# leggedrobotics/wild_visual_navigation

Measured on NVIDIA H100. Metric: frames/sec end-to-end (DINO feat + seg + MLP train-step) at 448x448, higher is better.
Workload: dtype bf16 operands / fp32 accumulate (ViT, STEGO head, per-pixel MLP); fp32 (k-means, train step)

## Files before the change

include/wvn_b200.h:

```cpp
#ifndef WVN_B200_H_
#define WVN_B200_H_

#include <stddef.h>
#include <stdint.h>

#ifdef __cplusplus
extern "C" {
#endif

typedef enum {
  WVN_STATUS_OK = 0,
  WVN_STATUS_INVALID = -1,
  WVN_STATUS_CUDA = -2,
  WVN_STATUS_NO_DEVICE = -3,
  WVN_STATUS_STATE = -4
} wvn_status;

const char* wvn_last_error(void);
int wvn_check_device(void);
int wvn_version(void);
long long wvn_launch_count(void);
void wvn_profile_enable(int category_mask);
int wvn_profile_collect(float* host_ms, long long* host_launches);

int wvn_gemm_bf16(const void* a_bf16, long long lda, const void* w_bf16, const float* bias, void* out, long long ldo,
                  int m, int n, int k, int out_kind, int act, int block_n, void* stream);

typedef struct {
  int m, n, k;
  int epi, act;
  int block_n;
  const void* a;
  long long lda;
  const void* w;
  const float* bias;
  void* out;
  long long ldo;
  const float* pos;
  int tokens_in, npad;
  int dim, heads;
  void* q_out;
  void* k_out;
  void* vt_out;
  int feat, trav_col;
  const void* x;
  long long ldx;
  float* trav;
  float* conf;
  float* loss_reco;
  const float* cg_mean;
  const float* cg_std;
  float cg_std_factor;
  int reverse_m;
  int registers;
  const void* residual;
  long long ldr;
} wvn_gemm_ex_args;
int wvn_gemm_bf16_ex(const wvn_gemm_ex_args* args, void* stream);

int wvn_attention_bf16(const void* q, const void* k, const void* vt, void* out, int batch, int heads, int npad,
                       int n_valid, float scale, void* stream);

int wvn_layernorm(const float* x, const float* gamma, const float* beta, void* out_bf16, long long rows, int dim,
                  float eps, void* stream);

typedef struct wvn_vit wvn_vit_t;

typedef struct {
  int image_size;
  int patch_size;
  int dim;
  int depth;
  int heads;
  int mlp_dim;
  int max_batch;
  int chunk;
  float ln_eps;
  int head_out;
  int registers;
} wvn_vit_config;

int wvn_vit_create(const wvn_vit_config* cfg, wvn_vit_t** out);
void wvn_vit_destroy(wvn_vit_t* h);

int wvn_vit_set_weight(wvn_vit_t* h, const char* name, const float* data, long long numel);

int wvn_vit_forward(wvn_vit_t* h, const float* img, int batch, int in_h, int in_w, int resized_h, int resized_w,
                    float* tokens_out, void* stream);

int wvn_vit_forward_tta(wvn_vit_t* h, const float* img, int batch, int in_h, int in_w, int resized_h, int resized_w,
                        float* tokens_out, void* stream);

int wvn_vit_forward_u8(wvn_vit_t* h, const unsigned char* img_hwc, int batch, int in_h, int in_w, int resized_h,
                       int resized_w, float* tokens_out, void* stream);

int wvn_vit_stego_head(wvn_vit_t* h, int batch, float* out, void* stream);
int wvn_vit_npad(const wvn_vit_t* h);

typedef struct wvn_resnet wvn_resnet_t;

typedef struct {
  int image_size;
  int depth;
  int max_batch;
} wvn_resnet_config;

int wvn_resnet_create(const wvn_resnet_config* cfg, wvn_resnet_t** out);
void wvn_resnet_destroy(wvn_resnet_t* h);
size_t wvn_resnet_workspace_bytes(const wvn_resnet_t* h);
int wvn_resnet_set_weight(wvn_resnet_t* h, const char* name, const float* data, long long numel);
int wvn_resnet_forward(wvn_resnet_t* h, const float* img, int batch, void* const* taps, void* stream);
// ... 160 lines not shown
```

wild_visual_navigation_b200/_C.py:

```python
from __future__ import annotations

import ctypes
import os
from ctypes import POINTER, Structure, byref, c_char_p, c_float, c_int, c_longlong, c_size_t, c_void_p

import torch

_HERE = os.path.dirname(os.path.abspath(__file__))
LIB_PATH = os.environ.get("WVN_B200_LIB", os.path.join(_HERE, "libwvn_b200.so"))


class WvnError(RuntimeError):
    pass


class VitConfig(Structure):
    _fields_ = [
        ("image_size", c_int), ("patch_size", c_int), ("dim", c_int), ("depth", c_int), ("heads", c_int),
        ("mlp_dim", c_int), ("max_batch", c_int), ("chunk", c_int), ("ln_eps", c_float), ("head_out", c_int),
        ("registers", c_int),
    ]


class GemmExArgs(Structure):
    _fields_ = [
        ("m", c_int), ("n", c_int), ("k", c_int), ("epi", c_int), ("act", c_int), ("block_n", c_int),
        ("a", c_void_p), ("lda", c_longlong), ("w", c_void_p), ("bias", c_void_p), ("out", c_void_p), ("ldo", c_longlong),
        ("pos", c_void_p), ("tokens_in", c_int), ("npad", c_int), ("dim", c_int), ("heads", c_int),
        ("q_out", c_void_p), ("k_out", c_void_p), ("vt_out", c_void_p),
        ("feat", c_int), ("trav_col", c_int), ("x", c_void_p), ("ldx", c_longlong), ("trav", c_void_p),
        ("conf", c_void_p), ("loss_reco", c_void_p), ("cg_mean", c_void_p), ("cg_std", c_void_p),
        ("cg_std_factor", c_float), ("reverse_m", c_int), ("registers", c_int), ("residual", c_void_p), ("ldr", c_longlong),
    ]


class ResnetConfig(Structure):
    _fields_ = [("image_size", c_int), ("depth", c_int), ("max_batch", c_int)]


class TrainConfig(Structure):
    _fields_ = [
        ("w_trav", c_float), ("w_reco", c_float), ("std_factor", c_float), ("anomaly_balanced", c_int),
        ("lr", c_float), ("beta1", c_float), ("beta2", c_float), ("eps", c_float),
    ]


class FlowBuffers(Structure):
    _fields_ = [("mask0", c_void_p), ("mask1", c_void_p), ("p1", c_void_p), ("invp1", c_void_p), ("p3", c_void_p),
                ("invp3", c_void_p)]


_lib = None

_P, _I, _L, _F, _S = c_void_p, c_int, c_longlong, c_float, c_size_t
SIGNATURES = {
    "wvn_last_error": (c_char_p, []),
    "wvn_check_device": (_I, []),
    "wvn_version": (_I, []),
    "wvn_launch_count": (_L, []),
    "wvn_profile_enable": (None, [_I]),
    "wvn_profile_collect": (_I, [_P, _P]),
    "wvn_gemm_bf16": (_I, [_P, _L, _P, _P, _P, _L, _I, _I, _I, _I, _I, _I, _P]),
    "wvn_gemm_bf16_ex": (_I, [POINTER(GemmExArgs), _P]),
    "wvn_attention_bf16": (_I, [_P, _P, _P, _P, _I, _I, _I, _I, _F, _P]),
    "wvn_layernorm": (_I, [_P, _P, _P, _P, _L, _I, _F, _P]),
    "wvn_vit_create": (_I, [POINTER(VitConfig), POINTER(_P)]),
    "wvn_vit_destroy": (None, [_P]),
    "wvn_vit_set_weight": (_I, [_P, c_char_p, _P, _L]),
    "wvn_vit_forward": (_I, [_P, _P, _I, _I, _I, _I, _I, _P, _P]),
    "wvn_vit_forward_u8": (_I, [_P, _P, _I, _I, _I, _I, _I, _P, _P]),
    "wvn_vit_forward_tta": (_I, [_P, _P, _I, _I, _I, _I, _I, _P, _P]),
    "wvn_vit_stego_head": (_I, [_P, _I, _P, _P]),
    "wvn_vit_npad": (_I, [_P]),
    "wvn_resnet_create": (_I, [POINTER(ResnetConfig), POINTER(_P)]),
    "wvn_resnet_destroy": (None, [_P]),
    "wvn_resnet_workspace_bytes": (_S, [_P]),
    "wvn_resnet_set_weight": (_I, [_P, c_char_p, _P, _L]),
    "wvn_resnet_forward": (_I, [_P, _P, _I, _P, _P]),
    "wvn_im2col_bf16_nhwc": (_I, [_P, _I, _I, _I, _I, _I, _I, _I, _P, _L, _P]),
    "wvn_im2col_image": (_I, [_P, _I, _I, _I, _I, _I, _I, _P, _L, _P]),
    "wvn_maxpool3s2_bf16_nhwc": (_I, [_P, _I, _I, _I, _I, _P, _P]),
    "wvn_segment_pool_pyramid": (_I, [_P, _I, _I, _I, _I, _P, _P, _P, _P, _P, _P, _P]),
    "wvn_upsample_dense": (_I, [_P, _P, _I, _I, _I, _I, _I, _I, _P]),
    "wvn_logits_argmax": (_I, [_P, _L, _I, _I, _I, _I, _I, _I, _I, _I, _I, _I, _P, _P, _P]),
    "wvn_flip_average": (_I, [_P, _I, _I, _I, _L, _P]),
    "wvn_stego_kmeans_workspace_bytes": (_S, [_I, _I, _I]),
    "wvn_stego_kmeans": (_I, [_P, _L, _I, _I, _I, _I, _I, _I, _I, _I, _P, _P, _P]),
    "wvn_segment_workspace_bytes": (_S, [_I, _I, _I, _I]),
    "wvn_segment_reduce": (_I, [_P, _I, _I, _I, _I, _P, _I, _I, _I, _P, _P, _P, _P, _I, _P, _P]),
    "wvn_segment_relabel": (_I, [_P, _I, _L, _I, _P, _P, _P]),
    "wvn_supervision_pool": (_I, [_P, _P, _I, _I, _I, _I, _I, _P, _P, _P, _P]),
    "wvn_slic_tables": (None, [_P, _P, _P]),
    "wvn_slic_geometry": (_I, [_I, _I, _I, _P, _P, _P]),
    "wvn_slic_workspace_bytes": (_S, [_I, _I, _I, _I]),
    "wvn_slic": (_I, [_P, _I, _I, _I, _I, _F, _I, _P, _P, _P, _P, _P, _P]),
    "wvn_project_and_render": (_I, [_P, _P, _P, _P, _I, _I, _I, _I, _I, _P, _P, _P, _P, _P, _P]),
    "wvn_mission_propagate_workspace_bytes": (_S, [_I, _I]),
    "wvn_mission_propagate": (_I, [_P, _P, _I, _P, _P, _P, _I, _P, _P, _P, _I, _I, _I, _P, _P, _P, _P, _P]),
    "wvn_mlp_infer_create": (_I, [_I, _I, _I, _I, POINTER(_P)]),
    "wvn_mlp_infer_destroy": (None, [_P]),
    "wvn_mlp_infer_reserve": (_I, [_P, _I]),
    "wvn_mlp_infer_set_params": (_I, [_P, _P, _P]),
    "wvn_mlp_infer_pixels": (_I, [_P, _P, _I, _I, _I, _I, _I, _P, _P, _F, _P, _P, _P]),
    "wvn_mlp_infer_pixels_vit": (_I, [_P, _P, _I, _I, _I, _P, _P, _F, _P, _P, _P]),
    "wvn_mlp_infer_rows": (_I, [_P, _P, _L, _P, _P, _F, _P, _P, _P]),
    "wvn_mlp_infer_create_double": (_I, [_I, _I, _I, _I, POINTER(_P)]),
    "wvn_mlp_param_count": (_S, [_I, _I, _I]),
    "wvn_mlp_train_workspace_bytes": (_S, [_I, _I, _I, _I]),
    "wvn_mlp_train_scalars_bytes": (_S, []),
    "wvn_mlp_train_forward_stats": (_I, [_I, _I, _I, _P, _P, _P, _P, _I, _I, _P, _P, _P]),
    "wvn_mlp_train_backward": (_I, [_I, _I, _I, _P, _P, _P, _P, _I, _I, _L, POINTER(TrainConfig), _P, _P, _P, _P, _P, _P, _P]),
    "wvn_mlp_train_apply": (_I, [_I, _I, _I, _P, _P, _P, _P, _P, _L, POINTER(TrainConfig), _P, _P]),
    "wvn_mlp_train_read_metrics": (_I, [_P, _P, _P]),
    "wvn_mlp_forward_f32": (_I, [_I, _I, _I, _P, _P, _I, _P, _P, _P, _P]),
    "wvn_trainer_destroy": (None, [_P]),
    "wvn_trainer_set_confidence": (_I, [_P, _I, _P, _P, _P, _P, _F, _F]),
# ... 69 lines not shown
```

wild_visual_navigation_b200/csrc/api.cu:

```cuda
#include <cuda_bf16.h>

#include <stdio.h>
#include <stdlib.h>

#include <map>
#include <string>
#include <vector>

#include "../../include/wvn_b200.h"
#include "attention.h"
#include "dense_kernels.h"
#include "double_mlp_train.h"
#include "gcn_train.h"
#include "gemm.h"
#include "host_common.h"
#include "mlp_train.h"
#include "mission_graph.h"
#include "mlp_train_fused.h"
#include "pixel_head.h"
#include "resnet_kernels.h"
#include "segment_kernels.h"
#include "flow_train.h"
#include "footprint_kernels.h"
#include "slic_kernels.h"
// ... 70 lines not shown
  bool forwarded = false;
  int last_batch = 0;

  int add_weight(const std::string& name, long long numel, bool bf16, int cols = 0, int ld = 0) {
    DevBuf b;
    const long long stored = cols > 0 ? numel / cols * ld : numel;
    WVN_PROPAGATE(b.alloc(static_cast<size_t>(stored) * (bf16 ? 2 : 4)));
    owned.push_back(b);
    Weight wt;
    wt.p = b.p; wt.numel = numel; wt.bf16 = bf16; wt.cols = cols; wt.ld = ld;
    w[name] = wt;
    return WVN_OK;
  }
  template <class T>
  T* wp(const std::string& name) { return reinterpret_cast<T*>(w[name].p); }
};

extern "C" {

const char* wvn_last_error(void) { return last_error(); }
int wvn_version(void) { return 108; }

int wvn_check_device(void) {
  int n = 0;
  if (cudaGetDeviceCount(&n) != cudaSuccess || n == 0) return set_error(WVN_ERR_NO_DEVICE, "no CUDA device visible");
  int dev = 0;
  cudaGetDevice(&dev);
  int major = 0;
  cudaDeviceGetAttribute(&major, cudaDevAttrComputeCapabilityMajor, dev);
  int minor = 0;
  cudaDeviceGetAttribute(&minor, cudaDevAttrComputeCapabilityMinor, dev);
  if (major != 9 || minor != 0)
    return set_error(WVN_ERR_NO_DEVICE, "device %d has compute capability %d.%d, need 9.0 (sm_90a)", dev, major, minor);
  return WVN_OK;
}

long long wvn_launch_count(void) { return launch_count(); }
void wvn_profile_enable(int category_mask) { prof_enable(category_mask); }
int wvn_profile_collect(float* host_ms, long long* host_launches) {
  WVN_REQUIRE(host_ms && host_launches, "wvn_profile_collect: null argument");
  return prof_collect(host_ms, host_launches);
}

int wvn_gemm_bf16(const void* a, long long lda, const void* w, const float* bias, void* out, long long ldo, int m, int n,
                  int k, int out_kind, int act, int block_n, void* stream) {
  GemmArgs g;
  g.M = m; g.N = n; g.K = k;
  g.epi = out_kind == 0 ? EPI_BF16 : (out_kind == 1 ? EPI_F32 : EPI_RESID_F32);
  WVN_REQUIRE(out_kind >= 0 && out_kind <= 2, "wvn_gemm_bf16: out_kind %d", out_kind);
  g.act = act; g.bias = bias; g.out = out; g.ldo = ldo;
  return gemm_bf16(g, a, lda, w, block_n, S(stream));
}

int wvn_gemm_bf16_ex(const wvn_gemm_ex_args* x, void* stream) {
  WVN_REQUIRE(x, "wvn_gemm_bf16_ex: null argument");
  GemmArgs g;
  g.M = x->m; g.N = x->n; g.K = x->k; g.epi = x->epi; g.act = x->act;
  g.bias = x->bias; g.out = x->out; g.ldo = x->ldo;
  g.pos = x->pos; g.tokens_in = x->tokens_in; g.npad = x->npad;
  g.dim = x->dim; g.heads = x->heads; g.q = x->q_out; g.k = x->k_out; g.vt = x->vt_out;
  g.feat = x->feat; g.trav_col = x->trav_col; g.x = x->x; g.ldx = x->ldx; g.trav = x->trav; g.conf = x->conf;
  g.loss_reco = x->loss_reco; g.cg_mean = x->cg_mean; g.cg_std = x->cg_std; g.cg_std_factor = x->cg_std_factor;
  g.reverse_m = x->reverse_m; g.registers = x->registers;
  g.residual = x->residual; g.ldr = x->ldr;
  return gemm_bf16(g, x->a, x->lda, x->w, x->block_n, S(stream));
}

int wvn_attention_bf16(const void* q, const void* k, const void* vt, void* out, int batch, int heads, int npad,
                       int n_valid, float scale, void* stream) {
  AttnArgs a;
  a.batch = batch; a.heads = heads; a.npad = npad; a.n_valid = n_valid;
  a.scale_log2 = scale * 1.4426950408889634f;
  a.out = out; a.ldo = static_cast<long long>(heads) * 64;
  return attention_bf16(a, q, k, vt, S(stream));
}

int wvn_layernorm(const float* x, const float* gamma, const float* beta, void* out_bf16, long long rows, int dim,
                  float eps, void* stream) {
  LayerNormArgs a;
  a.rows = rows; a.dim = dim; a.eps = eps;
  return layernorm_rows(x, gamma, beta, out_bf16, nullptr, a, S(stream));
}

int wvn_vit_create(const wvn_vit_config* cfg, wvn_vit_t** out) {
  WVN_REQUIRE(cfg && out, "wvn_vit_create: null argument");
  WVN_PROPAGATE(wvn_check_device());
  WVN_REQUIRE(cfg->dim == 384 || cfg->dim == 768, "vit: dim %d unsupported (384, 768)", cfg->dim);
  WVN_REQUIRE(cfg->heads * 64 == cfg->dim, "vit: heads*64 must equal dim");
  WVN_REQUIRE(cfg->patch_size == 8 || cfg->patch_size == 14 || cfg->patch_size == 16, "vit: patch size %d unsupported",
              cfg->patch_size);
  WVN_REQUIRE(cfg->image_size >= cfg->patch_size, "vit: image size too small");
  WVN_REQUIRE(cfg->mlp_dim % 64 == 0 && cfg->depth > 0 && cfg->max_batch > 0, "vit: bad mlp_dim/depth/max_batch");
  WVN_REQUIRE(cfg->head_out % 64 == 0, "vit: head_out must be a multiple of 64");
  WVN_REQUIRE(cfg->registers >= 0, "vit: registers must be >= 0");
  WVN_REQUIRE(cfg->registers == 0 || cfg->head_out == 0, "vit: register tokens and a STEGO head cannot be combined");
  wvn_vit* h = new wvn_vit();
  h->cfg = *cfg;
  if (h->cfg.ln_eps <= 0.f) h->cfg.ln_eps = 1e-6f;
  h->grid = cfg->image_size / cfg->patch_size;
  h->P = h->grid * h->grid;
  h->t0 = 1 + cfg->registers;
  h->n_valid = h->t0 + h->P;
  h->npad = round_up(h->n_valid, 128);
  h->kpe = 3 * cfg->patch_size * cfg->patch_size;
  h->kpe_ld = patch_pitch(cfg->patch_size);
  h->chunk = cfg->chunk > 0 ? cfg->chunk : 8;
  if (h->chunk > cfg->max_batch) h->chunk = cfg->max_batch;
  const int D = cfg->dim;
  int rc = WVN_OK;
  auto add = [&](const std::string& n, long long numel, bool bf) { if (rc == WVN_OK) rc = h->add_weight(n, numel, bf); };
  add("cls_token", D, false);
  add("pos_embed", static_cast<long long>(1 + h->P) * D, false);
  if (cfg->registers > 0) add("register_tokens", static_cast<long long>(cfg->registers) * D, false);
  if (rc == WVN_OK) rc = h->add_weight("patch_embed.proj.weight", static_cast<long long>(D) * h->kpe, true, h->kpe, h->kpe_ld);
  add("patch_embed.proj.bias", D, false);
  for (int i = 0; i < cfg->depth; ++i) {
    const std::string b = "blocks." + std::to_string(i) + ".";
    add(b + "norm1.weight", D, false);
// ... 1276 lines not shown
```

wild_visual_navigation_b200/csrc/gemm.h:

```cpp
#pragma once

#include <cuda_runtime.h>

namespace wvn {

enum GemmEpilogue : int {
  EPI_BF16 = 0,
  EPI_F32 = 1,
  EPI_RESID_F32 = 2,
  EPI_PATCH = 3,
  EPI_QKV = 4,
  EPI_MLP_HEAD = 5,
  EPI_BF16_RESID = 6,
};

enum GemmAct : int { ACT_NONE = 0, ACT_RELU = 1, ACT_GELU = 2 };

struct GemmArgs {
  int M = 0, N = 0, K = 0;
  int epi = EPI_BF16, act = ACT_NONE;
  const float* bias = nullptr;
  void* out = nullptr;
  long long ldo = 0;
  const float* pos = nullptr;
  int tokens_in = 0;
  int registers = 0;
  int npad = 0;
  int dim = 0, heads = 0;
  void* q = nullptr;
  void* k = nullptr;
  void* vt = nullptr;
  int feat = 0;
  int trav_col = 0;
  const void* x = nullptr;
  long long ldx = 0;
  float* trav = nullptr;
  float* conf = nullptr;
  float* loss_reco = nullptr;
  const float* cg_mean = nullptr;
  const float* cg_std = nullptr;
  float cg_std_factor = 0.5f;
  const void* residual = nullptr;
  long long ldr = 0;
  int max_ctas = 0;
  int reverse_m = 0;
};

int pick_block_n(int N);

inline long long gemm_w_pitch(int K) { return (static_cast<long long>(K) + 7) / 8 * 8; }

int gemm_bf16(const GemmArgs& args, const void* A, long long lda, const void* W, int block_n, cudaStream_t stream);

}
```

wild_visual_navigation_b200/csrc/gemm_wgmma.cu:

```cuda
#include <stdlib.h>

#include <algorithm>

#include "common.cuh"
#include "gemm.h"
#include "host_common.h"

namespace wvn {

namespace {

constexpr int BM = 64;
constexpr int BK = 64;
constexpr int kConsumerWarps = 8;
constexpr int kNumThreads = 128 + kConsumerWarps * 32;
constexpr int kMaxSmemBytes = 227 * 1024;
constexpr int kMaxStages = 8;
constexpr int kFixedSmemBytes = 1024  + 1024 ;
constexpr int kSliceCols = 32;
constexpr int kResidMaxBlockN = 192;

template <bool ROW_OWNER>
struct TileIter {
  int num_m, num_n, m_blk, n_blk, lin;
  __device__ TileIter(int nm, int nn) : num_m(nm), num_n(nn), m_blk(0), n_blk(0), lin(0) {
    if (ROW_OWNER) { m_blk = blockIdx.x; n_blk = 0; }
    else { lin = blockIdx.x; m_blk = lin / num_n; n_blk = lin % num_n; }
  }
  __device__ bool valid() const { return m_blk < num_m; }
  __device__ void next() {
    if (ROW_OWNER) { if (++n_blk == num_n) { n_blk = 0; m_blk += gridDim.x; } }
    else { lin += gridDim.x; m_blk = lin / num_n; n_blk = lin % num_n; }
  }
};

template <int EPI>
constexpr bool kStaged = EPI == EPI_BF16 || EPI == EPI_F32 || EPI == EPI_RESID_F32 || EPI == EPI_QKV || EPI == EPI_BF16_RESID;

template <int BN, int EPI>
struct GemmCfg {
  static constexpr uint32_t kABytes = BM * BK * 2;
  static constexpr uint32_t kBBytes = BN * BK * 2;
  static constexpr uint32_t kStageBytes = kABytes + kBBytes;
  static constexpr uint32_t kSliceBytes = BM * kSliceCols * ((EPI == EPI_F32 || EPI == EPI_RESID_F32) ? 4 : 2);
  static constexpr uint32_t kStagingBytes = kStaged<EPI> ? 2 * 2 * kSliceBytes : 0;
  static constexpr int kStagesRaw = (kMaxSmemBytes - kFixedSmemBytes - kStagingBytes) / kStageBytes;
  static constexpr int kStages = kStagesRaw > kMaxStages ? kMaxStages : kStagesRaw;
  static constexpr uint32_t kSmemBytes = kStages * kStageBytes + kStagingBytes + kFixedSmemBytes;
  static constexpr int kN128 = BN / 128;
  static constexpr int kN64 = (BN % 128) / 64;
  static constexpr int kN32 = (BN % 64) / 32;
};

__device__ __forceinline__ float gelu_erf_fast(float x) {
  const float t = fminf(fabsf(x), 5.5f);
  float p = fmaf(-0.0003865310864f, t, 0.006509808358f);
  p = fmaf(p, t, -0.05048002675f);
  p = fmaf(p, t, -0.4613505006f);
  p = fmaf(p, t, -1.150225043f);
  p = fmaf(p, t, -1.00010848f);
  float e;
  asm("ex2.approx.ftz.f32 %0, %1;" : "=f"(e) : "f"(p));
  return fmaf(-t, e, fmaxf(x, 0.f));
}

template <int ACT>
__device__ __forceinline__ float activate(float v) {
  if (ACT == ACT_RELU) return fmaxf(v, 0.f);
  if (ACT == ACT_GELU) return gelu_erf_fast(v);
  return v;
}

template <int EPI, int ACT, int NREG>
__device__ __forceinline__ void epilogue_frag(const GemmArgs& args, const float (&d)[NREG], const int row0,
                                              const int col_base, const int lane, float (&head_partial)[2]) {
  const int q = lane & 3;
  bool ok[2];
  long long orow[2];
  int tok[2];
#pragma unroll
  for (int h = 0; h < 2; ++h) {
    const int row = row0 + 8 * h;
    ok[h] = row < args.M;
    orow[h] = row;
    tok[h] = 0;
    if (EPI == EPI_PATCH) {
      const int frame = row / args.tokens_in;
      tok[h] = row - frame * args.tokens_in;
      orow[h] = static_cast<long long>(frame) * args.npad + (1 + args.registers) + tok[h];
    }
  }
#pragma unroll
  for (int j = 0; j < NREG / 4; ++j) {
    const int col = col_base + 8 * j + 2 * q;
    float2 b = make_float2(0.f, 0.f);
    if (args.bias != nullptr) b = __ldg(reinterpret_cast<const float2*>(args.bias + col));
#pragma unroll
    for (int h = 0; h < 2; ++h) {
      const float v0 = activate<ACT>(d[4 * j + 2 * h] + b.x), v1 = activate<ACT>(d[4 * j + 2 * h + 1] + b.y);
      if (!ok[h]) continue;
      if (EPI == EPI_PATCH) {
// ... 34 lines not shown
    if (leader) {
      if (si == 0) tma_store_wait_read<0>();
      else tma_store_wait_read<1>();
    }
    named_bar_sync(bar_id, 128);
#pragma unroll
    for (int js = 0; js < 4; ++js) {
      const int j = 4 * s + js;
      const int c = col + 8 * js + 2 * q;
      float2 b = make_float2(0.f, 0.f);
      if (args.bias != nullptr) b = __ldg(reinterpret_cast<const float2*>(args.bias + c));
#pragma unroll
      for (int h = 0; h < 2; ++h) {
        const int r = row_local + 8 * h;
        float a0 = d[4 * j + 2 * h] + b.x, a1 = d[4 * j + 2 * h + 1] + b.y;
        if (EPI == EPI_BF16_RESID && row_tile + r < args.M) {
          const uint32_t rv = __ldg(reinterpret_cast<const uint32_t*>(
              reinterpret_cast<const __nv_bfloat16*>(args.residual) + static_cast<long long>(row_tile + r) * args.ldr + c));
          a0 += bf16_lo(rv);
          a1 += bf16_hi(rv);
        }
        const float v0 = activate<ACT>(a0), v1 = activate<ACT>(a1);
        if (EPI == EPI_F32 || EPI == EPI_RESID_F32) {
          sts64(buf + r * 128 + ((((2 * js + (q >> 1)) ^ (r & 7))) << 4) + (q & 1) * 8, v0, v1);
        } else if (EPI == EPI_QKV && which == 2) {
          const int dd = 8 * js + 2 * q;
          const uint32_t t = 2 * r;
          sts16(buf + dd * 128 + (((t >> 4) ^ (dd & 7)) << 4) + (t & 15), __float2bfloat16_rn(v0));
          sts16(buf + (dd + 1) * 128 + (((t >> 4) ^ ((dd + 1) & 7)) << 4) + (t & 15), __float2bfloat16_rn(v1));
        } else {
          sts32(buf + r * 64 + ((js ^ ((r >> 1) & 3)) << 4) + q * 4, pack_bf16x2(v0, v1));
        }
      }
    }
    fence_proxy_async_smem();
    named_bar_sync(bar_id, 128);
    if (leader) {
      if (EPI == EPI_BF16 || EPI == EPI_F32 || EPI == EPI_BF16_RESID) {
        tma_store_2d(tm0, buf, col, row_tile);
      } else if (EPI == EPI_RESID_F32) {
        tma_reduce_add_2d(tm0, buf, col, row_tile);
      } else if (EPI == EPI_QKV) {
        const int frame = row_tile / args.npad;
        const int tok0 = row_tile - frame * args.npad;
        const int bh = frame * args.heads + (within >> 6);
        if (which < 2) tma_store_2d(which == 0 ? tm0 : tm1, buf, within & 63, bh * args.npad + tok0);
        else tma_store_2d(tm2, buf, tok0, bh * 64 + (within & 63));
      }
      tma_store_commit();
    }
  }
}

template <int BN, int EPI, int ACT>
__global__ void __launch_bounds__(kNumThreads, 1)
gemm_bf16_kernel(const __grid_constant__ CUtensorMap tmap_a, const __grid_constant__ CUtensorMap tmap_b,
                 const __grid_constant__ CUtensorMap tmap_c0, const __grid_constant__ CUtensorMap tmap_c1,
                 const __grid_constant__ CUtensorMap tmap_c2, const GemmArgs args) {
  using Cfg = GemmCfg<BN, EPI>;
  constexpr int STAGES = Cfg::kStages;

  extern __shared__ uint8_t smem_raw[];
  uint8_t* smem = reinterpret_cast<uint8_t*>((reinterpret_cast<uintptr_t>(smem_raw) + 1023) & ~uintptr_t(1023));
  uint8_t* smem_b = smem;
  uint8_t* smem_a = smem + STAGES * Cfg::kBBytes;
  uint8_t* smem_c = smem_a + STAGES * Cfg::kABytes;
  uint64_t* bars = reinterpret_cast<uint64_t*>(smem_c + Cfg::kStagingBytes);
  uint64_t* full_bar = bars;
  uint64_t* empty_bar = bars + kMaxStages;

  const int warp = threadIdx.x >> 5;
  const int lane = threadIdx.x & 31;

  const int num_m = (args.M + BM - 1) / BM;
  const int num_n = args.N / BN;
  const int num_k = (args.K + BK - 1) / BK;
  constexpr bool ROW_OWNER = (EPI == EPI_MLP_HEAD);

  if (threadIdx.x == 0) {
    tma_prefetch_desc(&tmap_a);
    tma_prefetch_desc(&tmap_b);
    for (int i = 0; i < kMaxStages; ++i) {
      mbar_init(&full_bar[i], 1);
      mbar_init(&empty_bar[i], kConsumerWarps / 2);
    }
    fence_mbar_init();
  }
  __syncthreads();

  if (warp < 4) {
    setmaxnreg_dec<40>();
    if (warp == 0) {
      int stage = 0;
      uint32_t phase = 0;
      for (TileIter<ROW_OWNER> it(num_m, num_n); it.valid(); it.next()) {
        const int m_eff = args.reverse_m ? num_m - 1 - it.m_blk : it.m_blk;
        for (int kb = 0; kb < num_k; ++kb) {
          mbar_wait(&empty_bar[stage], phase ^ 1);
          if (elect_one_sync()) {
            mbar_arrive_expect_tx(&full_bar[stage], Cfg::kStageBytes);
            tma_load_2d(&tmap_a, &full_bar[stage], smem_a + stage * Cfg::kABytes, kb * BK, m_eff * BM);
            tma_load_2d(&tmap_b, &full_bar[stage], smem_b + stage * Cfg::kBBytes, kb * BK, it.n_blk * BN);
          }
          __syncwarp();
          if (++stage == STAGES) { stage = 0; phase ^= 1; }
        }
      }
    }
  } else {
    setmaxnreg_inc<232>();
    const int cwarp = warp - 4;
    const int wg = cwarp >> 2;
    const int row_local = (cwarp & 3) * 16 + (lane >> 2);
    const bool leader = (threadIdx.x & 127) == 0;
    const uint32_t staging = smem_u32(smem_c) + wg * 2 * Cfg::kSliceBytes;
    if (kStaged<EPI> && leader) {
      tma_prefetch_desc(&tmap_c0);
      if (EPI == EPI_QKV) {
        tma_prefetch_desc(&tmap_c1);
        tma_prefetch_desc(&tmap_c2);
      }
    }
    if (wg == 1) named_bar_arrive(1, 256);
    float acc128[Cfg::kN128 > 0 ? Cfg::kN128 : 1][64];
    float acc64[32];
    float acc32[16];
    float head_partial[2] = {0.f, 0.f};
    int stage = 0;
    uint32_t phase = 0;
    int unit = 0;
    for (TileIter<ROW_OWNER> it(num_m, num_n); it.valid(); it.next()) {
      const bool unit_end = !ROW_OWNER || it.n_blk == num_n - 1;
      if ((unit & 1) != wg) {
        for (int kb = 0; kb < num_k; ++kb)
          if (++stage == STAGES) { stage = 0; phase ^= 1; }
        if (unit_end) ++unit;
        continue;
      }
      if (!ROW_OWNER || it.n_blk == 0) named_bar_sync(1 + wg, 256);
      int prev_stage = 0;
      for (int kb = 0; kb < num_k; ++kb) {
        mbar_wait(&full_bar[stage], phase);
        const uint64_t desc_a = make_sw128_kmajor_desc(smem_u32(smem_a + stage * Cfg::kABytes));
        const uint32_t b_addr = smem_u32(smem_b + stage * Cfg::kBBytes);
#pragma unroll
        for (int c = 0; c < Cfg::kN128; ++c) wgmma_fence_regs(acc128[c]);
        if (Cfg::kN64) wgmma_fence_regs(acc64);
        if (Cfg::kN32) wgmma_fence_regs(acc32);
        wgmma_fence();
#pragma unroll
        for (int k = 0; k < BK / 16; ++k) {
          const uint32_t accumulate = (kb | k) != 0 ? 1u : 0u;
#pragma unroll
          for (int c = 0; c < Cfg::kN128; ++c)
            wgmma_m64n128k16_ss(acc128[c], desc_a + 2 * k, make_sw128_kmajor_desc(b_addr + c * 128 * 128) + 2 * k, accumulate);
          if (Cfg::kN64)
            wgmma_m64n64k16_ss(acc64, desc_a + 2 * k, make_sw128_kmajor_desc(b_addr + Cfg::kN128 * 128 * 128) + 2 * k, accumulate);
          if (Cfg::kN32)
            wgmma_m64n32k16_ss(acc32, desc_a + 2 * k,
                               make_sw128_kmajor_desc(b_addr + (Cfg::kN128 * 128 + Cfg::kN64 * 64) * 128) + 2 * k, accumulate);
        }
        wgmma_commit();
        if (kb > 0) {
          wgmma_wait<1>();
          if (lane == 0) mbar_arrive(&empty_bar[prev_stage]);
        }
        prev_stage = stage;
        if (++stage == STAGES) { stage = 0; phase ^= 1; }
      }
      if (unit_end && (ROW_OWNER ? it.m_blk + static_cast<int>(gridDim.x) < num_m : it.lin + static_cast<int>(gridDim.x) < num_m * num_n))
        named_bar_arrive(2 - wg, 256);
      wgmma_wait<0>();
#pragma unroll
      for (int c = 0; c < Cfg::kN128; ++c) wgmma_fence_regs(acc128[c]);
      if (Cfg::kN64) wgmma_fence_regs(acc64);
      if (Cfg::kN32) wgmma_fence_regs(acc32);
      if (lane == 0) mbar_arrive(&empty_bar[prev_stage]);

      const int m_eff = args.reverse_m ? num_m - 1 - it.m_blk : it.m_blk;
      const int row_tile = m_eff * BM;
      const int col0 = it.n_blk * BN;
      if (kStaged<EPI>) {
        const int bar_id = 3 + wg;
#pragma unroll
        for (int c = 0; c < Cfg::kN128; ++c)
          store_frag<EPI, ACT>(args, &tmap_c0, &tmap_c1, &tmap_c2, acc128[c], row_tile, col0 + c * 128, row_local, lane,
                               leader, bar_id, staging, Cfg::kSliceBytes, 4 * c);
        if (Cfg::kN64)
          store_frag<EPI, ACT>(args, &tmap_c0, &tmap_c1, &tmap_c2, acc64, row_tile, col0 + Cfg::kN128 * 128, row_local,
                               lane, leader, bar_id, staging, Cfg::kSliceBytes, 4 * Cfg::kN128);
        if (Cfg::kN32)
          store_frag<EPI, ACT>(args, &tmap_c0, &tmap_c1, &tmap_c2, acc32, row_tile, col0 + Cfg::kN128 * 128 + Cfg::kN64 * 64,
                               row_local, lane, leader, bar_id, staging, Cfg::kSliceBytes, 4 * Cfg::kN128 + 2 * Cfg::kN64);
      } else {
        const int row0 = row_tile + row_local;
#pragma unroll
        for (int c = 0; c < Cfg::kN128; ++c)
          epilogue_frag<EPI, ACT>(args, acc128[c], row0, col0 + c * 128, lane, head_partial);
        if (Cfg::kN64) epilogue_frag<EPI, ACT>(args, acc64, row0, col0 + Cfg::kN128 * 128, lane, head_partial);
        if (Cfg::kN32) epilogue_frag<EPI, ACT>(args, acc32, row0, col0 + Cfg::kN128 * 128 + Cfg::kN64 * 64, lane, head_partial);
      }

      if (EPI == EPI_MLP_HEAD && it.n_blk == num_n - 1) {
#pragma unroll
        for (int h = 0; h < 2; ++h) {
          float s = head_partial[h];
          s += __shfl_xor_sync(0xffffffffu, s, 1);
          s += __shfl_xor_sync(0xffffffffu, s, 2);
          head_partial[h] = 0.f;
          const int row = row_tile + row_local + 8 * h;
          if ((lane & 3) == 0 && row < args.M) {
            const float loss = s / static_cast<float>(args.feat);
            const float mean = __ldg(args.cg_mean), sd = __ldg(args.cg_std);
            const float shifted = mean + sd * args.cg_std_factor;
            const float lo = fmaxf(shifted - sd, 0.f);
            const float hi = shifted + sd;
            const float xc = fminf(fmaxf(loss, lo), hi);
            args.conf[row] = 1.f - (xc - lo) / (hi - lo);
            if (args.loss_reco != nullptr) args.loss_reco[row] = loss;
          }
        }
      }
      if (unit_end) ++unit;
    }
    if (kStaged<EPI> && leader) tma_store_wait_all<0>();
  }
}

template <int BN, int EPI, int ACT>
int launch_gemm(const GemmArgs& a, const CUtensorMap& ta, const CUtensorMap& tb, const CUtensorMap (&tc)[3],
                cudaStream_t stream) {
  using Cfg = GemmCfg<BN, EPI>;
  static_assert(Cfg::kStages >= 2, "tile too wide for the shared-memory budget");
  auto kern = gemm_bf16_kernel<BN, EPI, ACT>;
  static bool attr_set = false;
  if (!attr_set) {
    WVN_CHECK_CUDA(cudaFuncSetAttribute(kern, cudaFuncAttributeMaxDynamicSharedMemorySize, kMaxSmemBytes));
    attr_set = true;
  }
  const int num_m = (a.M + BM - 1) / BM, num_n = a.N / BN;
  const int num_tiles = (EPI == EPI_MLP_HEAD) ? num_m : num_m * num_n;
  int grid = sm_count();
  if (a.max_ctas > 0 && a.max_ctas < grid) grid = a.max_ctas;
  if (grid > num_tiles) grid = num_tiles;
  prof_begin(PROF_GEMM, stream);
  kern<<<grid, kNumThreads, Cfg::kSmemBytes, stream>>>(ta, tb, tc[0], tc[1], tc[2], a);
  prof_end(PROF_GEMM, stream);
  WVN_CHECK_LAUNCH("gemm_bf16_kernel");
  return WVN_OK;
}

template <int BN>
int dispatch_epi(const GemmArgs& a, const CUtensorMap& ta, const CUtensorMap& tb, const CUtensorMap (&tc)[3],
                 cudaStream_t s) {
  switch (a.epi) {
    case EPI_BF16:
      if (a.act == ACT_NONE) return launch_gemm<BN, EPI_BF16, ACT_NONE>(a, ta, tb, tc, s);
      if (a.act == ACT_RELU) return launch_gemm<BN, EPI_BF16, ACT_RELU>(a, ta, tb, tc, s);
      if (a.act == ACT_GELU) return launch_gemm<BN, EPI_BF16, ACT_GELU>(a, ta, tb, tc, s);
      break;
    case EPI_F32:
      if (a.act == ACT_NONE) return launch_gemm<BN, EPI_F32, ACT_NONE>(a, ta, tb, tc, s);
      break;
    case EPI_RESID_F32:
      if (a.act == ACT_NONE) return launch_gemm<BN, EPI_RESID_F32, ACT_NONE>(a, ta, tb, tc, s);
      break;
    case EPI_PATCH:
      if (a.act == ACT_NONE) return launch_gemm<BN, EPI_PATCH, ACT_NONE>(a, ta, tb, tc, s);
      break;
    case EPI_QKV:
      if (a.act == ACT_NONE) return launch_gemm<BN, EPI_QKV, ACT_NONE>(a, ta, tb, tc, s);
      break;
    case EPI_MLP_HEAD:
      if (a.act == ACT_NONE) return launch_gemm<BN, EPI_MLP_HEAD, ACT_NONE>(a, ta, tb, tc, s);
      break;
    case EPI_BF16_RESID:
      if constexpr (BN <= kResidMaxBlockN) {
        if (a.act == ACT_NONE) return launch_gemm<BN, EPI_BF16_RESID, ACT_NONE>(a, ta, tb, tc, s);
        if (a.act == ACT_RELU) return launch_gemm<BN, EPI_BF16_RESID, ACT_RELU>(a, ta, tb, tc, s);
      }
      break;
  }
  return set_error(WVN_ERR_INVALID, "gemm: unsupported epilogue/activation combination (%d, %d)", a.epi, a.act);
}

}

int pick_block_n(int N) {
  if (N % 256 == 0) return 256;
  if (N % 224 == 0) return 224;
  if (N % 192 == 0) return 192;
  if (N % 128 == 0) return 128;
  if (N % 64 == 0) return 64;
  return 0;
}

int gemm_bf16(const GemmArgs& a, const void* A, long long lda, const void* W, int block_n, cudaStream_t stream) {
  WVN_REQUIRE(a.M > 0 && a.N > 0 && a.K > 0, "gemm: empty problem (M=%d N=%d K=%d)", a.M, a.N, a.K);
  WVN_REQUIRE(lda >= a.K, "gemm: lda=%lld is smaller than K=%d", lda, a.K);
  if (block_n == 0) {
    block_n = pick_block_n(a.N);
    if (a.epi == EPI_BF16_RESID && block_n > kResidMaxBlockN) block_n = a.N % 192 == 0 ? 192 : (a.N % 128 == 0 ? 128 : 64);
  }
  WVN_REQUIRE(a.epi != EPI_BF16_RESID || block_n <= kResidMaxBlockN, "gemm: the residual epilogue takes block_n <= %d",
              kResidMaxBlockN);
  WVN_REQUIRE(block_n == 64 || block_n == 128 || block_n == 192 || block_n == 224 || block_n == 256,
              "gemm: bad block_n %d", block_n);
  WVN_REQUIRE(a.N % block_n == 0, "gemm: N=%d must be a multiple of block_n=%d (pad the weights)", a.N, block_n);
  if (a.epi == EPI_MLP_HEAD)
    WVN_REQUIRE(a.feat > 0 && a.trav_col % 32 == 0 && a.trav_col >= a.feat && a.trav_col < a.N && a.x != nullptr &&
                    a.trav != nullptr && a.conf != nullptr && a.cg_mean != nullptr && a.cg_std != nullptr &&
                    a.ldx % 8 == 0 && a.ldx >= a.trav_col,
                "gemm: bad MLP-head epilogue arguments (feat=%d trav_col=%d N=%d)", a.feat, a.trav_col, a.N);
  if (a.epi == EPI_QKV)
    WVN_REQUIRE(a.dim % 64 == 0 && a.N == 3 * a.dim && a.heads * 64 == a.dim && a.npad % 8 == 0 && a.npad % BM == 0 &&
                    a.M % a.npad == 0,
                "gemm: bad QKV epilogue geometry (dim=%d heads=%d npad=%d N=%d M=%d)", a.dim, a.heads, a.npad, a.N, a.M);
  if (a.epi == EPI_PATCH)
    WVN_REQUIRE(a.tokens_in > 0 && a.registers >= 0 && 1 + a.registers + a.tokens_in <= a.npad,
                "gemm: bad patch-embed epilogue geometry (tokens_in=%d registers=%d npad=%d)", a.tokens_in, a.registers,
                a.npad);
  if (a.epi == EPI_F32 || a.epi == EPI_RESID_F32) WVN_REQUIRE(a.ldo % 4 == 0, "gemm: fp32 output pitch must be a multiple of 4");
  if (a.epi == EPI_BF16 || a.epi == EPI_BF16_RESID) WVN_REQUIRE(a.ldo % 8 == 0, "gemm: bf16 output pitch must be a multiple of 8");
  if (a.epi == EPI_BF16_RESID)
    WVN_REQUIRE(a.residual != nullptr && a.ldr >= a.N && a.ldr % 2 == 0,
                "gemm: the residual epilogue needs a bf16 residual with an even pitch ldr >= N (ldr=%lld N=%d)", a.ldr, a.N);
  CUtensorMap ta, tb, tc[3] = {};
  WVN_PROPAGATE(make_tmap_bf16_2d(&ta, A, a.K, a.M, static_cast<uint64_t>(lda) * 2, BK, BM));
  WVN_PROPAGATE(make_tmap_bf16_2d(&tb, W, a.K, a.N, static_cast<uint64_t>(gemm_w_pitch(a.K)) * 2, BK, block_n));
  if (a.epi == EPI_BF16 || a.epi == EPI_BF16_RESID)
    WVN_PROPAGATE(make_tmap_2d(&tc[0], a.out, 2, a.N, a.M, static_cast<uint64_t>(a.ldo) * 2, kSliceCols, BM, 64));
  if (a.epi == EPI_F32 || a.epi == EPI_RESID_F32)
    WVN_PROPAGATE(make_tmap_2d(&tc[0], a.out, 4, a.N, a.M, static_cast<uint64_t>(a.ldo) * 4, kSliceCols, BM, 128));
  if (a.epi == EPI_QKV) {
    const uint64_t bh = static_cast<uint64_t>(a.M / a.npad) * a.heads;
    WVN_PROPAGATE(make_tmap_2d(&tc[0], a.q, 2, 64, bh * a.npad, 128, kSliceCols, BM, 64));
    WVN_PROPAGATE(make_tmap_2d(&tc[1], a.k, 2, 64, bh * a.npad, 128, kSliceCols, BM, 64));
    WVN_PROPAGATE(make_tmap_2d(&tc[2], a.vt, 2, a.npad, bh * 64, static_cast<uint64_t>(a.npad) * 2, BM, kSliceCols, 128));
  }
  switch (block_n) {
    case 64: return dispatch_epi<64>(a, ta, tb, tc, stream);
    case 128: return dispatch_epi<128>(a, ta, tb, tc, stream);
    case 192: return dispatch_epi<192>(a, ta, tb, tc, stream);
    case 224: return dispatch_epi<224>(a, ta, tb, tc, stream);
    case 256: return dispatch_epi<256>(a, ta, tb, tc, stream);
  }
  return set_error(WVN_ERR_INVALID, "gemm: unreachable");
}

}
```

Baseline: 970.7.

## Keep GEMM weight slab resident in shared memory for K=384 persistent tiles

Adds a slab mode to the persistent wgmma GEMM for problems whose K spans exactly six k-blocks. Each CTA is pinned to one N-block, loads that block's full weight panel into shared memory once via TMA, and then streams only A tiles across its assigned M-blocks. The intent is to stop re-fetching B tiles every k-step, which shrinks per-stage TMA traffic and frees pipeline bytes for A. In exchange the pipeline has fewer stages and the grid is rounded to a multiple of the slab count, which can leave SMs idle or unbalance the tiles.

```diff
diff --git a/include/wvn_b200.h b/include/wvn_b200.h
--- a/include/wvn_b200.h
+++ b/include/wvn_b200.h
@@ -57,6 +57,8 @@
   long long ldr;
 } wvn_gemm_ex_args;
 int wvn_gemm_bf16_ex(const wvn_gemm_ex_args* args, void* stream);
+int wvn_gemm_bf16_ex_ctas(const wvn_gemm_ex_args* args, int max_ctas, void* stream);
+int wvn_gemm_plan(int m, int n, int k, int epi, int act, int block_n, int max_ctas, int sm_count, int* plan);
 
 int wvn_attention_bf16(const void* q, const void* k, const void* vt, void* out, int batch, int heads, int npad,
                        int n_valid, float scale, void* stream);
diff --git a/wild_visual_navigation_b200/_C.py b/wild_visual_navigation_b200/_C.py
--- a/wild_visual_navigation_b200/_C.py
+++ b/wild_visual_navigation_b200/_C.py
@@ -62,6 +62,8 @@
     "wvn_profile_collect": (_I, [_P, _P]),
     "wvn_gemm_bf16": (_I, [_P, _L, _P, _P, _P, _L, _I, _I, _I, _I, _I, _I, _P]),
     "wvn_gemm_bf16_ex": (_I, [POINTER(GemmExArgs), _P]),
+    "wvn_gemm_bf16_ex_ctas": (_I, [POINTER(GemmExArgs), _I, _P]),
+    "wvn_gemm_plan": (_I, [_I, _I, _I, _I, _I, _I, _I, _I, _P]),
     "wvn_attention_bf16": (_I, [_P, _P, _P, _P, _I, _I, _I, _I, _F, _P]),
     "wvn_layernorm": (_I, [_P, _P, _P, _P, _L, _I, _F, _P]),
     "wvn_vit_create": (_I, [POINTER(VitConfig), POINTER(_P)]),
diff --git a/wild_visual_navigation_b200/csrc/api.cu b/wild_visual_navigation_b200/csrc/api.cu
--- a/wild_visual_navigation_b200/csrc/api.cu
+++ b/wild_visual_navigation_b200/csrc/api.cu
@@ -146,9 +146,13 @@
   return gemm_bf16(g, a, lda, w, block_n, S(stream));
 }
 
-int wvn_gemm_bf16_ex(const wvn_gemm_ex_args* x, void* stream) {
+int wvn_gemm_bf16_ex(const wvn_gemm_ex_args* x, void* stream) { return wvn_gemm_bf16_ex_ctas(x, 0, stream); }
+
+int wvn_gemm_bf16_ex_ctas(const wvn_gemm_ex_args* x, int max_ctas, void* stream) {
   WVN_REQUIRE(x, "wvn_gemm_bf16_ex: null argument");
+  WVN_REQUIRE(max_ctas >= 0, "wvn_gemm_bf16_ex_ctas: max_ctas %d", max_ctas);
   GemmArgs g;
+  g.max_ctas = max_ctas;
   g.M = x->m; g.N = x->n; g.K = x->k; g.epi = x->epi; g.act = x->act;
   g.bias = x->bias; g.out = x->out; g.ldo = x->ldo;
   g.pos = x->pos; g.tokens_in = x->tokens_in; g.npad = x->npad;
@@ -158,6 +162,15 @@
   g.reverse_m = x->reverse_m; g.registers = x->registers;
   g.residual = x->residual; g.ldr = x->ldr;
   return gemm_bf16(g, x->a, x->lda, x->w, x->block_n, S(stream));
+}
+
+int wvn_gemm_plan(int m, int n, int k, int epi, int act, int block_n, int max_ctas, int sms, int* plan) {
+  WVN_REQUIRE(plan && m > 0 && n > 0 && k > 0 && sms > 0 && max_ctas >= 0, "wvn_gemm_plan: bad argument");
+  GemmArgs g;
+  g.M = m; g.N = n; g.K = k; g.epi = epi; g.act = act; g.max_ctas = max_ctas;
+  const GemmPlan p = gemm_plan(g, block_n, sms);
+  plan[0] = p.block_n; plan[1] = p.slab; plan[2] = p.grid;
+  return WVN_OK;
 }
 
 int wvn_attention_bf16(const void* q, const void* k, const void* vt, void* out, int batch, int heads, int npad,
diff --git a/wild_visual_navigation_b200/csrc/gemm.h b/wild_visual_navigation_b200/csrc/gemm.h
--- a/wild_visual_navigation_b200/csrc/gemm.h
+++ b/wild_visual_navigation_b200/csrc/gemm.h
@@ -48,6 +48,13 @@
 
 int pick_block_n(int N);
 
+struct GemmPlan {
+  int block_n = 0;
+  int slab = 0;
+  int grid = 0;
+};
+GemmPlan gemm_plan(const GemmArgs& args, int block_n, int sms);
+
 inline long long gemm_w_pitch(int K) { return (static_cast<long long>(K) + 7) / 8 * 8; }
 
 int gemm_bf16(const GemmArgs& args, const void* A, long long lda, const void* W, int block_n, cudaStream_t stream);
diff --git a/wild_visual_navigation_b200/csrc/gemm_wgmma.cu b/wild_visual_navigation_b200/csrc/gemm_wgmma.cu
--- a/wild_visual_navigation_b200/csrc/gemm_wgmma.cu
+++ b/wild_visual_navigation_b200/csrc/gemm_wgmma.cu
@@ -19,8 +19,10 @@
 constexpr int kFixedSmemBytes = 1024  + 1024 ;
 constexpr int kSliceCols = 32;
 constexpr int kResidMaxBlockN = 192;
-
-template <bool ROW_OWNER>
+constexpr int kSlabKBlocks = 6;
+constexpr int kSlabMinStages = 4;
+
+template <bool ROW_OWNER, bool SLAB>
 struct TileIter {
   int num_m, num_n, m_blk, n_blk, lin;
   __device__ TileIter(int nm, int nn) : num_m(nm), num_n(nn), m_blk(0), n_blk(0), lin(0) {
@@ -30,23 +32,31 @@
   __device__ bool valid() const { return m_blk < num_m; }
   __device__ void next() {
     if (ROW_OWNER) { if (++n_blk == num_n) { n_blk = 0; m_blk += gridDim.x; } }
+    else if (SLAB) { m_blk += gridDim.x / num_n; }
     else { lin += gridDim.x; m_blk = lin / num_n; n_blk = lin % num_n; }
+  }
+  __device__ bool more() const {
+    if (ROW_OWNER) return m_blk + static_cast<int>(gridDim.x) < num_m;
+    if (SLAB) return m_blk + static_cast<int>(gridDim.x) / num_n < num_m;
+    return lin + static_cast<int>(gridDim.x) < num_m * num_n;
   }
 };
 
 template <int EPI>
 constexpr bool kStaged = EPI == EPI_BF16 || EPI == EPI_F32 || EPI == EPI_RESID_F32 || EPI == EPI_QKV || EPI == EPI_BF16_RESID;
 
-template <int BN, int EPI>
+template <int BN, int EPI, bool SLAB = false>
 struct GemmCfg {
   static constexpr uint32_t kABytes = BM * BK * 2;
   static constexpr uint32_t kBBytes = BN * BK * 2;
-  static constexpr uint32_t kStageBytes = kABytes + kBBytes;
+  static constexpr uint32_t kSlabBytes = SLAB ? kSlabKBlocks * kBBytes : 0;
+  static constexpr uint32_t kStageBytes = SLAB ? kABytes : kABytes + kBBytes;
   static constexpr uint32_t kSliceBytes = BM * kSliceCols * ((EPI == EPI_F32 || EPI == EPI_RESID_F32) ? 4 : 2);
   static constexpr uint32_t kStagingBytes = kStaged<EPI> ? 2 * 2 * kSliceBytes : 0;
-  static constexpr int kStagesRaw = (kMaxSmemBytes - kFixedSmemBytes - kStagingBytes) / kStageBytes;
+  static constexpr int kStagesRaw =
+      (static_cast<int>(kMaxSmemBytes - kFixedSmemBytes - kStagingBytes) - static_cast<int>(kSlabBytes)) / static_cast<int>(kStageBytes);
   static constexpr int kStages = kStagesRaw > kMaxStages ? kMaxStages : kStagesRaw;
-  static constexpr uint32_t kSmemBytes = kStages * kStageBytes + kStagingBytes + kFixedSmemBytes;
+  static constexpr uint32_t kSmemBytes = kSlabBytes + kStages * kStageBytes + kStagingBytes + kFixedSmemBytes;
   static constexpr int kN128 = BN / 128;
   static constexpr int kN64 = (BN % 128) / 64;
   static constexpr int kN32 = (BN % 64) / 32;
@@ -187,22 +197,23 @@
   }
 }
 
-template <int BN, int EPI, int ACT>
+template <int BN, int EPI, int ACT, bool SLAB>
 __global__ void __launch_bounds__(kNumThreads, 1)
 gemm_bf16_kernel(const __grid_constant__ CUtensorMap tmap_a, const __grid_constant__ CUtensorMap tmap_b,
                  const __grid_constant__ CUtensorMap tmap_c0, const __grid_constant__ CUtensorMap tmap_c1,
                  const __grid_constant__ CUtensorMap tmap_c2, const GemmArgs args) {
-  using Cfg = GemmCfg<BN, EPI>;
+  using Cfg = GemmCfg<BN, EPI, SLAB>;
   constexpr int STAGES = Cfg::kStages;
 
   extern __shared__ uint8_t smem_raw[];
   uint8_t* smem = reinterpret_cast<uint8_t*>((reinterpret_cast<uintptr_t>(smem_raw) + 1023) & ~uintptr_t(1023));
   uint8_t* smem_b = smem;
-  uint8_t* smem_a = smem + STAGES * Cfg::kBBytes;
+  uint8_t* smem_a = smem + (SLAB ? Cfg::kSlabBytes : STAGES * Cfg::kBBytes);
   uint8_t* smem_c = smem_a + STAGES * Cfg::kABytes;
   uint64_t* bars = reinterpret_cast<uint64_t*>(smem_c + Cfg::kStagingBytes);
   uint64_t* full_bar = bars;
   uint64_t* empty_bar = bars + kMaxStages;
+  uint64_t* slab_bar = bars + 2 * kMaxStages;
 
   const int warp = threadIdx.x >> 5;
   const int lane = threadIdx.x & 31;
@@ -219,6 +230,7 @@
       mbar_init(&full_bar[i], 1);
       mbar_init(&empty_bar[i], kConsumerWarps / 2);
     }
+    mbar_init(slab_bar, 1);
     fence_mbar_init();
   }
   __syncthreads();
@@ -228,14 +240,22 @@
     if (warp == 0) {
       int stage = 0;
       uint32_t phase = 0;
-      for (TileIter<ROW_OWNER> it(num_m, num_n); it.valid(); it.next()) {
+      if (SLAB && TileIter<ROW_OWNER, SLAB>(num_m, num_n).valid()) {
+        if (elect_one_sync()) {
+          mbar_arrive_expect_tx(slab_bar, num_k * Cfg::kBBytes);
+          for (int kb = 0; kb < num_k; ++kb)
+            tma_load_2d(&tmap_b, slab_bar, smem_b + kb * Cfg::kBBytes, kb * BK, (blockIdx.x % num_n) * BN);
+        }
+        __syncwarp();
+      }
+      for (TileIter<ROW_OWNER, SLAB> it(num_m, num_n); it.valid(); it.next()) {
         const int m_eff = args.reverse_m ? num_m - 1 - it.m_blk : it.m_blk;
         for (int kb = 0; kb < num_k; ++kb) {
           mbar_wait(&empty_bar[stage], phase ^ 1);
           if (elect_one_sync()) {
             mbar_arrive_expect_tx(&full_bar[stage], Cfg::kStageBytes);
             tma_load_2d(&tmap_a, &full_bar[stage], smem_a + stage * Cfg::kABytes, kb * BK, m_eff * BM);
-            tma_load_2d(&tmap_b, &full_bar[stage], smem_b + stage * Cfg::kBBytes, kb * BK, it.n_blk * BN);
+            if (!SLAB) tma_load_2d(&tmap_b, &full_bar[stage], smem_b + stage * Cfg::kBBytes, kb * BK, it.n_blk * BN);
           }
           __syncwarp();
           if (++stage == STAGES) { stage = 0; phase ^= 1; }
@@ -264,7 +284,7 @@
     int stage = 0;
     uint32_t phase = 0;
     int unit = 0;
-    for (TileIter<ROW_OWNER> it(num_m, num_n); it.valid(); it.next()) {
+    for (TileIter<ROW_OWNER, SLAB> it(num_m, num_n); it.valid(); it.next()) {
       const bool unit_end = !ROW_OWNER || it.n_blk == num_n - 1;
       if ((unit & 1) != wg) {
         for (int kb = 0; kb < num_k; ++kb)
@@ -273,11 +293,12 @@
         continue;
       }
       if (!ROW_OWNER || it.n_blk == 0) named_bar_sync(1 + wg, 256);
+      if (SLAB) mbar_wait(slab_bar, 0);
       int prev_stage = 0;
       for (int kb = 0; kb < num_k; ++kb) {
         mbar_wait(&full_bar[stage], phase);
         const uint64_t desc_a = make_sw128_kmajor_desc(smem_u32(smem_a + stage * Cfg::kABytes));
-        const uint32_t b_addr = smem_u32(smem_b + stage * Cfg::kBBytes);
+        const uint32_t b_addr = smem_u32(smem_b + (SLAB ? kb : stage) * Cfg::kBBytes);
 #pragma unroll
         for (int c = 0; c < Cfg::kN128; ++c) wgmma_fence_regs(acc128[c]);
         if (Cfg::kN64) wgmma_fence_regs(acc64);
@@ -303,8 +324,7 @@
         prev_stage = stage;
         if (++stage == STAGES) { stage = 0; phase ^= 1; }
       }
-      if (unit_end && (ROW_OWNER ? it.m_blk + static_cast<int>(gridDim.x) < num_m : it.lin + static_cast<int>(gridDim.x) < num_m * num_n))
-        named_bar_arrive(2 - wg, 256);
+      if (unit_end && it.more()) named_bar_arrive(2 - wg, 256);
       wgmma_wait<0>();
 #pragma unroll
       for (int c = 0; c < Cfg::kN128; ++c) wgmma_fence_regs(acc128[c]);
@@ -362,22 +382,17 @@
   }
 }
 
-template <int BN, int EPI, int ACT>
-int launch_gemm(const GemmArgs& a, const CUtensorMap& ta, const CUtensorMap& tb, const CUtensorMap (&tc)[3],
+template <int BN, int EPI, int ACT, bool SLAB>
+int launch_gemm(const GemmArgs& a, const CUtensorMap& ta, const CUtensorMap& tb, const CUtensorMap (&tc)[3], int grid,
                 cudaStream_t stream) {
-  using Cfg = GemmCfg<BN, EPI>;
-  static_assert(Cfg::kStages >= 2, "tile too wide for the shared-memory budget");
-  auto kern = gemm_bf16_kernel<BN, EPI, ACT>;
+  using Cfg = GemmCfg<BN, EPI, SLAB>;
+  static_assert(Cfg::kStages >= (SLAB ? kSlabMinStages : 2), "tile too wide for the shared-memory budget");
+  auto kern = gemm_bf16_kernel<BN, EPI, ACT, SLAB>;
   static bool attr_set = false;
   if (!attr_set) {
     WVN_CHECK_CUDA(cudaFuncSetAttribute(kern, cudaFuncAttributeMaxDynamicSharedMemorySize, kMaxSmemBytes));
     attr_set = true;
   }
-  const int num_m = (a.M + BM - 1) / BM, num_n = a.N / BN;
-  const int num_tiles = (EPI == EPI_MLP_HEAD) ? num_m : num_m * num_n;
-  int grid = sm_count();
-  if (a.max_ctas > 0 && a.max_ctas < grid) grid = a.max_ctas;
-  if (grid > num_tiles) grid = num_tiles;
   prof_begin(PROF_GEMM, stream);
   kern<<<grid, kNumThreads, Cfg::kSmemBytes, stream>>>(ta, tb, tc[0], tc[1], tc[2], a);
   prof_end(PROF_GEMM, stream);
@@ -386,33 +401,46 @@
 }
 
 template <int BN>
-int dispatch_epi(const GemmArgs& a, const CUtensorMap& ta, const CUtensorMap& tb, const CUtensorMap (&tc)[3],
+int dispatch_slab(const GemmArgs& a, const CUtensorMap& ta, const CUtensorMap& tb, const CUtensorMap (&tc)[3], int grid,
+                  cudaStream_t s) {
+  if (a.epi == EPI_QKV && a.act == ACT_NONE) return launch_gemm<BN, EPI_QKV, ACT_NONE, true>(a, ta, tb, tc, grid, s);
+  if (a.epi == EPI_RESID_F32 && a.act == ACT_NONE) return launch_gemm<BN, EPI_RESID_F32, ACT_NONE, true>(a, ta, tb, tc, grid, s);
+  if (a.epi == EPI_BF16) {
+    if (a.act == ACT_NONE) return launch_gemm<BN, EPI_BF16, ACT_NONE, true>(a, ta, tb, tc, grid, s);
+    if (a.act == ACT_RELU) return launch_gemm<BN, EPI_BF16, ACT_RELU, true>(a, ta, tb, tc, grid, s);
+    if (a.act == ACT_GELU) return launch_gemm<BN, EPI_BF16, ACT_GELU, true>(a, ta, tb, tc, grid, s);
+  }
+  return set_error(WVN_ERR_INVALID, "gemm: no slab kernel for epilogue/activation (%d, %d)", a.epi, a.act);
+}
+
+template <int BN>
+int dispatch_epi(const GemmArgs& a, const CUtensorMap& ta, const CUtensorMap& tb, const CUtensorMap (&tc)[3], int grid,
                  cudaStream_t s) {
   switch (a.epi) {
     case EPI_BF16:
-      if (a.act == ACT_NONE) return launch_gemm<BN, EPI_BF16, ACT_NONE>(a, ta, tb, tc, s);
-      if (a.act == ACT_RELU) return launch_gemm<BN, EPI_BF16, ACT_RELU>(a, ta, tb, tc, s);
-      if (a.act == ACT_GELU) return launch_gemm<BN, EPI_BF16, ACT_GELU>(a, ta, tb, tc, s);
+      if (a.act == ACT_NONE) return launch_gemm<BN, EPI_BF16, ACT_NONE, false>(a, ta, tb, tc, grid, s);
+      if (a.act == ACT_RELU) return launch_gemm<BN, EPI_BF16, ACT_RELU, false>(a, ta, tb, tc, grid, s);
+      if (a.act == ACT_GELU) return launch_gemm<BN, EPI_BF16, ACT_GELU, false>(a, ta, tb, tc, grid, s);
       break;
     case EPI_F32:
-      if (a.act == ACT_NONE) return launch_gemm<BN, EPI_F32, ACT_NONE>(a, ta, tb, tc, s);
+      if (a.act == ACT_NONE) return launch_gemm<BN, EPI_F32, ACT_NONE, false>(a, ta, tb, tc, grid, s);
       break;
     case EPI_RESID_F32:
-      if (a.act == ACT_NONE) return launch_gemm<BN, EPI_RESID_F32, ACT_NONE>(a, ta, tb, tc, s);
+      if (a.act == ACT_NONE) return launch_gemm<BN, EPI_RESID_F32, ACT_NONE, false>(a, ta, tb, tc, grid, s);
       break;
     case EPI_PATCH:
-      if (a.act == ACT_NONE) return launch_gemm<BN, EPI_PATCH, ACT_NONE>(a, ta, tb, tc, s);
+      if (a.act == ACT_NONE) return launch_gemm<BN, EPI_PATCH, ACT_NONE, false>(a, ta, tb, tc, grid, s);
       break;
     case EPI_QKV:
-      if (a.act == ACT_NONE) return launch_gemm<BN, EPI_QKV, ACT_NONE>(a, ta, tb, tc, s);
+      if (a.act == ACT_NONE) return launch_gemm<BN, EPI_QKV, ACT_NONE, false>(a, ta, tb, tc, grid, s);
       break;
     case EPI_MLP_HEAD:
-      if (a.act == ACT_NONE) return launch_gemm<BN, EPI_MLP_HEAD, ACT_NONE>(a, ta, tb, tc, s);
+      if (a.act == ACT_NONE) return launch_gemm<BN, EPI_MLP_HEAD, ACT_NONE, false>(a, ta, tb, tc, grid, s);
       break;
     case EPI_BF16_RESID:
       if constexpr (BN <= kResidMaxBlockN) {
-        if (a.act == ACT_NONE) return launch_gemm<BN, EPI_BF16_RESID, ACT_NONE>(a, ta, tb, tc, s);
-        if (a.act == ACT_RELU) return launch_gemm<BN, EPI_BF16_RESID, ACT_RELU>(a, ta, tb, tc, s);
+        if (a.act == ACT_NONE) return launch_gemm<BN, EPI_BF16_RESID, ACT_NONE, false>(a, ta, tb, tc, grid, s);
+        if (a.act == ACT_RELU) return launch_gemm<BN, EPI_BF16_RESID, ACT_RELU, false>(a, ta, tb, tc, grid, s);
       }
       break;
   }
@@ -430,13 +458,54 @@
   return 0;
 }
 
+namespace {
+template <int BN, int EPI>
+constexpr bool slab_fits() { return GemmCfg<BN, EPI, true>::kStages >= kSlabMinStages; }
+
+bool slab_fits(int bn, int epi) {
+  if (epi == EPI_QKV) return bn == 128 ? slab_fits<128, EPI_QKV>() : slab_fits<192, EPI_QKV>();
+  if (epi == EPI_BF16) return bn == 128 ? slab_fits<128, EPI_BF16>() : slab_fits<192, EPI_BF16>();
+  if (epi == EPI_RESID_F32) return bn == 128 ? slab_fits<128, EPI_RESID_F32>() : slab_fits<192, EPI_RESID_F32>();
+  return false;
+}
+}
+
+GemmPlan gemm_plan(const GemmArgs& a, int block_n, int sms) {
+  static int slab_env = -1;
+  if (slab_env < 0) { const char* e = getenv("WVN_GEMM_SLAB"); slab_env = (e && atoi(e) == 0) ? 0 : 1; }
+  GemmPlan p;
+  const int cap = (a.max_ctas > 0 && a.max_ctas < sms) ? a.max_ctas : sms;
+  const int num_m = (a.M + BM - 1) / BM;
+  const bool slab_epi = a.epi == EPI_QKV || a.epi == EPI_BF16 || a.epi == EPI_RESID_F32;
+  if (block_n == 0 && slab_env && slab_epi && (a.K + BK - 1) / BK == kSlabKBlocks) {
+    for (const int bn : {192, 128}) {
+      const int slabs = a.N / bn;
+      if (a.N % bn != 0 || !slab_fits(bn, a.epi) || slabs > cap) continue;
+      if (p.slab == 0 || (sms % (a.N / p.block_n) != 0 && sms % slabs == 0)) { p.block_n = bn; p.slab = 1; }
+    }
+  }
+  if (p.slab) {
+    const int slabs = a.N / p.block_n;
+    p.grid = slabs * std::min(cap / slabs, num_m);
+    return p;
+  }
+  if (block_n == 0) {
+    block_n = pick_block_n(a.N);
+    if (a.epi == EPI_BF16_RESID && block_n > kResidMaxBlockN) block_n = a.N % 192 == 0 ? 192 : (a.N % 128 == 0 ? 128 : 64);
+  }
+  p.block_n = block_n;
+  if (block_n > 0 && a.N % block_n == 0) {
+    const int num_tiles = (a.epi == EPI_MLP_HEAD) ? num_m : num_m * (a.N / block_n);
+    p.grid = std::min(cap, num_tiles);
+  }
+  return p;
+}
+
 int gemm_bf16(const GemmArgs& a, const void* A, long long lda, const void* W, int block_n, cudaStream_t stream) {
   WVN_REQUIRE(a.M > 0 && a.N > 0 && a.K > 0, "gemm: empty problem (M=%d N=%d K=%d)", a.M, a.N, a.K);
   WVN_REQUIRE(lda >= a.K, "gemm: lda=%lld is smaller than K=%d", lda, a.K);
-  if (block_n == 0) {
-    block_n = pick_block_n(a.N);
-    if (a.epi == EPI_BF16_RESID && block_n > kResidMaxBlockN) block_n = a.N % 192 == 0 ? 192 : (a.N % 128 == 0 ? 128 : 64);
-  }
+  const GemmPlan plan = gemm_plan(a, block_n, sm_count());
+  block_n = plan.block_n;
   WVN_REQUIRE(a.epi != EPI_BF16_RESID || block_n <= kResidMaxBlockN, "gemm: the residual epilogue takes block_n <= %d",
               kResidMaxBlockN);
   WVN_REQUIRE(block_n == 64 || block_n == 128 || block_n == 192 || block_n == 224 || block_n == 256,
@@ -473,12 +542,14 @@
     WVN_PROPAGATE(make_tmap_2d(&tc[1], a.k, 2, 64, bh * a.npad, 128, kSliceCols, BM, 64));
     WVN_PROPAGATE(make_tmap_2d(&tc[2], a.vt, 2, a.npad, bh * 64, static_cast<uint64_t>(a.npad) * 2, BM, kSliceCols, 128));
   }
+  if (plan.slab) return block_n == 128 ? dispatch_slab<128>(a, ta, tb, tc, plan.grid, stream)
+                                        : dispatch_slab<192>(a, ta, tb, tc, plan.grid, stream);
   switch (block_n) {
-    case 64: return dispatch_epi<64>(a, ta, tb, tc, stream);
-    case 128: return dispatch_epi<128>(a, ta, tb, tc, stream);
-    case 192: return dispatch_epi<192>(a, ta, tb, tc, stream);
-    case 224: return dispatch_epi<224>(a, ta, tb, tc, stream);
-    case 256: return dispatch_epi<256>(a, ta, tb, tc, stream);
+    case 64: return dispatch_epi<64>(a, ta, tb, tc, plan.grid, stream);
+    case 128: return dispatch_epi<128>(a, ta, tb, tc, plan.grid, stream);
+    case 192: return dispatch_epi<192>(a, ta, tb, tc, plan.grid, stream);
+    case 224: return dispatch_epi<224>(a, ta, tb, tc, plan.grid, stream);
+    case 256: return dispatch_epi<256>(a, ta, tb, tc, plan.grid, stream);
   }
   return set_error(WVN_ERR_INVALID, "gemm: unreachable");
 }
```

New measurement: 994.9 (median of 6 runs). 1.03x the previous value.
